# Atticuszz/GsplatLoc

Measured on AMD Instinct MI355X. Metric: Gaussians/s fwd+bwd @1M splats 1200x680, higher is better.
Workload: dtype f32

## Files before the change

### gsplatloc_amd/csrc/gsloc_common.h

```cpp
#pragma once
#include <hip/hip_runtime.h>
#include <stdint.h>

#include "../../include/gsloc_hip.h"

#define GSL_WAVE 64
#define GSL_ALPHA_MAX 0.999f
#define GSL_ALPHA_MIN (1.0f / 255.0f)
#define GSL_T_STOP 1e-4f
#define GSL_LOG2E 1.4426950408889634f

#define GSL_CHECK_LAUNCH()                                   \
  do {                                                       \
    hipError_t e__ = hipGetLastError();                      \
    if (e__ != hipSuccess) return GSL_ERR_HIP;               \
  } while (0)

namespace gsl {

int zero_u32(void* p, size_t n_dwords, hipStream_t st);

struct M3 {
  float m[9];
  __device__ __forceinline__ float& operator()(int r, int c) { return m[r * 3 + c]; }
  __device__ __forceinline__ float operator()(int r, int c) const { return m[r * 3 + c]; }
};

__device__ __forceinline__ M3 mul(const M3& a, const M3& b) {
  M3 o;
#pragma unroll
  for (int i = 0; i < 3; ++i)
#pragma unroll
    for (int j = 0; j < 3; ++j)
      o(i, j) = a(i, 0) * b(0, j) + a(i, 1) * b(1, j) + a(i, 2) * b(2, j);
  return o;
}
__device__ __forceinline__ M3 mul_bt(const M3& a, const M3& b) {
  M3 o;
#pragma unroll
  for (int i = 0; i < 3; ++i)
#pragma unroll
    for (int j = 0; j < 3; ++j)
      o(i, j) = a(i, 0) * b(j, 0) + a(i, 1) * b(j, 1) + a(i, 2) * b(j, 2);
  return o;
}
__device__ __forceinline__ M3 mul_at(const M3& a, const M3& b) {
  M3 o;
#pragma unroll
  for (int i = 0; i < 3; ++i)
#pragma unroll
    for (int j = 0; j < 3; ++j)
      o(i, j) = a(0, i) * b(0, j) + a(1, i) * b(1, j) + a(2, i) * b(2, j);
  return o;
}

__device__ __forceinline__ M3 quat_to_rotmat(float w, float x, float y, float z) {
  float inv = rsqrtf(w * w + x * x + y * y + z * z);
  w *= inv; x *= inv; y *= inv; z *= inv;
  M3 R;
  R(0, 0) = 1.f - 2.f * (y * y + z * z); R(0, 1) = 2.f * (x * y - w * z); R(0, 2) = 2.f * (x * z + w * y);
  R(1, 0) = 2.f * (x * y + w * z); R(1, 1) = 1.f - 2.f * (x * x + z * z); R(1, 2) = 2.f * (y * z - w * x);
  R(2, 0) = 2.f * (x * z - w * y); R(2, 1) = 2.f * (y * z + w * x); R(2, 2) = 1.f - 2.f * (x * x + y * y);
  return R;
}

__device__ __forceinline__ M3 quat_scale_to_covar(const float q[4], const float s[3]) {
  M3 R = quat_to_rotmat(q[0], q[1], q[2], q[3]);
  M3 M;
#pragma unroll
  for (int i = 0; i < 3; ++i)
#pragma unroll
    for (int j = 0; j < 3; ++j) M(i, j) = R(i, j) * s[j];
  return mul_bt(M, M);
}

struct Cam {
  M3 R;
  float t[3];
  float fx, fy, cx, cy;
};

__device__ __forceinline__ Cam load_cam(const float* __restrict__ V, const float* __restrict__ K) {
  Cam c;
#pragma unroll
  for (int i = 0; i < 3; ++i) {
#pragma unroll
    for (int j = 0; j < 3; ++j) c.R(i, j) = V[i * 4 + j];
    c.t[i] = V[i * 4 + 3];
  }
  c.fx = K[0]; c.fy = K[4]; c.cx = K[2]; c.cy = K[5];
  return c;
}

#define GSL_Q(arr, g) (arr)[(g)]
#ifndef GSL_NG
#define GSL_NG 4
#endif
#define GSL_HIT_SHIFT (32 - GSL_NG)
#define GSL_HIT_INDEX_MASK ((1u << GSL_HIT_SHIFT) - 1u)
#define GSL_CLAMP_DEPTH_WINDOW(nearp, farp)            \
  do {                                                 \
    if (!((nearp) >= 1.17549435e-38f)) (nearp) = 1.17549435e-38f; \
    if (!((farp) <= 3.40282347e+38f)) (farp) = 3.40282347e+38f;   \
  } while (0)
#define GSL_MAX_GAUSSIANS (1 << 26)
#ifndef GSL_XCD_SPANS
#define GSL_XCD_SPANS 0
#endif
__device__ __forceinline__ int xcd_span_item(int b, int n) {
#if GSL_XCD_SPANS
  const int x = b & 7, k = b >> 3, q = n >> 3, r = n & 7;
  return x * q + min(x, r) + k;
#else
  (void)n;
  return b;
#endif
}
#define GSL_TILE_OF_BLOCK() gsl::xcd_span_item((int)blockIdx.x, (int)gridDim.x)

__device__ __forceinline__ unsigned pack2h(float a, float b) {
  _Float16 ha = (_Float16)a, hb = (_Float16)b;
  return (unsigned)__builtin_bit_cast(unsigned short, ha) | ((unsigned)__builtin_bit_cast(unsigned short, hb) << 16);
}
__device__ __forceinline__ float h_lo(unsigned u) { return (float)__builtin_bit_cast(_Float16, (unsigned short)(u & 0xFFFFu)); }
__device__ __forceinline__ float h_hi(unsigned u) { return (float)__builtin_bit_cast(_Float16, (unsigned short)(u >> 16)); }

__device__ __forceinline__ void store_half_record(uint4* __restrict__ Qh, size_t i, float4 q0, float4 q1, float4 q2) {
  float rc = (q1.w > 0.f && q1.w < 6.0e4f) ? q1.w * 1.002f + 0.01f : q1.w;
  Qh[2 * i] = make_uint4(__float_as_uint(q0.x), __float_as_uint(q0.y), pack2h(q1.x, q1.y), pack2h(q1.z, rc));
  Qh[2 * i + 1] = make_uint4(pack2h(0.f, q0.w), pack2h(q2.x, q2.y), pack2h(q2.z, 0.f), __float_as_uint(q0.z));
}

__device__ __forceinline__ void load_record(const float4* __restrict__ Q0, const float4* __restrict__ Q1,
                                            const float4* __restrict__ Q2, const uint4* __restrict__ Qh, int g,
                                            bool want_rgb, float4& r0, float4& r1, float4& r2) {
  if (Qh) {
    uint4 lo = Qh[2 * (size_t)g], hi = Qh[2 * (size_t)g + 1];
    r0 = make_float4(__uint_as_float(lo.x), __uint_as_float(lo.y), __uint_as_float(hi.w), h_hi(hi.x));
    r1 = make_float4(h_lo(lo.z), h_hi(lo.z), h_lo(lo.w), h_hi(lo.w));
    r2 = make_float4(h_lo(hi.y), h_hi(hi.y), h_lo(hi.z), 0.f);
  } else {
    r0 = GSL_Q(Q0, g);
    r1 = GSL_Q(Q1, g);
    if (want_rgb) r2 = GSL_Q(Q2, g);
  }
}

__device__ __forceinline__ int32_t list_id(const int32_t* __restrict__ storage_of, uint64_t key) {
  uint32_t g = (uint32_t)key;
  return storage_of ? storage_of[g] : (int32_t)g;
}

template <int CTRL, int ROW_MASK = 0xF>
__device__ __forceinline__ float dpp_get(float v) {
  return __builtin_bit_cast(
      float, __builtin_amdgcn_update_dpp(0, __builtin_bit_cast(int, v), CTRL, ROW_MASK, 0xF, true));
}

__device__ __forceinline__ float wave_sum(float v) {
  v += dpp_get<0xB1>(v);
  v += dpp_get<0x4E>(v);
  v += dpp_get<0x141>(v);
  v += dpp_get<0x140>(v);
  v += dpp_get<0x142, 0xA>(v);
  v += dpp_get<0x143, 0xC>(v);
  return __builtin_bit_cast(float, __builtin_amdgcn_readlane(__builtin_bit_cast(int, v), 63));
}

__device__ __forceinline__ void cam_inverse(const Cam& cam, M3& Ri, float cp[3]) {
  const M3& R = cam.R;
  float c00 = R(1, 1) * R(2, 2) - R(1, 2) * R(2, 1);
  float c01 = R(1, 2) * R(2, 0) - R(1, 0) * R(2, 2);
  float c02 = R(1, 0) * R(2, 1) - R(1, 1) * R(2, 0);
  float det = R(0, 0) * c00 + R(0, 1) * c01 + R(0, 2) * c02;
  float id = 1.f / det;
  Ri(0, 0) = c00 * id; Ri(1, 0) = c01 * id; Ri(2, 0) = c02 * id;
  Ri(0, 1) = (R(0, 2) * R(2, 1) - R(0, 1) * R(2, 2)) * id;
  Ri(1, 1) = (R(0, 0) * R(2, 2) - R(0, 2) * R(2, 0)) * id;
  Ri(2, 1) = (R(0, 1) * R(2, 0) - R(0, 0) * R(2, 1)) * id;
  Ri(0, 2) = (R(0, 1) * R(1, 2) - R(0, 2) * R(1, 1)) * id;
  Ri(1, 2) = (R(0, 2) * R(1, 0) - R(0, 0) * R(1, 2)) * id;
  Ri(2, 2) = (R(0, 0) * R(1, 1) - R(0, 1) * R(1, 0)) * id;
#pragma unroll
  for (int k = 0; k < 3; ++k) cp[k] = -(Ri(k, 0) * cam.t[0] + Ri(k, 1) * cam.t[1] + Ri(k, 2) * cam.t[2]);
}

__device__ __forceinline__ float viewmat_from_totals(const float* tot, const float* __restrict__ V,
                                                     const float* __restrict__ Kmat) {
  float v = 0.f;
  if (threadIdx.x < 16) {
    int r = threadIdx.x >> 2, c = threadIdx.x & 3;
    if (r < 3) {
      Cam cam = load_cam(V, Kmat);
      M3 Ri;
      float cp[3];
      cam_inverse(cam, Ri, cp);
      float w = Ri(0, r) * tot[12] + Ri(1, r) * tot[13] + Ri(2, r) * tot[14];
      if (c < 3) v = tot[r * 3 + c] - w * cp[c];
      else v = tot[9 + r] - w;
    }
  }
  return v;
}

__device__ __forceinline__ float reduce_viewmat_rows(const float* __restrict__ partials, int nb,
                                                     const float* __restrict__ V, const float* __restrict__ Kmat,
                                                     float (*red)[15], float* tot) {
  int q = threadIdx.x & 3;
  const float4* rows = reinterpret_cast<const float4*>(partials) + q;
  float4 a0 = make_float4(0.f, 0.f, 0.f, 0.f), a1 = a0, a2 = a0, a3 = a0;
  int b = threadIdx.x >> 2;
  for (; b + 192 < nb; b += 256) {
    float4 x0 = rows[(size_t)b * 4], x1 = rows[(size_t)(b + 64) * 4], x2 = rows[(size_t)(b + 128) * 4],
           x3 = rows[(size_t)(b + 192) * 4];
    a0.x += x0.x; a0.y += x0.y; a0.z += x0.z; a0.w += x0.w;
    a1.x += x1.x; a1.y += x1.y; a1.z += x1.z; a1.w += x1.w;
    a2.x += x2.x; a2.y += x2.y; a2.z += x2.z; a2.w += x2.w;
    a3.x += x3.x; a3.y += x3.y; a3.z += x3.z; a3.w += x3.w;
  }
  for (; b < nb; b += 64) {
    float4 x0 = rows[(size_t)b * 4];
    a0.x += x0.x; a0.y += x0.y; a0.z += x0.z; a0.w += x0.w;
  }
  float v4[4] = {(a0.x + a1.x) + (a2.x + a3.x), (a0.y + a1.y) + (a2.y + a3.y), (a0.z + a1.z) + (a2.z + a3.z),
                 (a0.w + a1.w) + (a2.w + a3.w)};
  int lane = threadIdx.x & 63, wv = threadIdx.x >> 6;
#pragma unroll
  for (int c = 0; c < 4; ++c) {
    float x = v4[c];
#pragma unroll
    for (int o = 4; o < 64; o <<= 1) x += __shfl_xor(x, o, 64);
    if (lane < 4 && 4 * q + c < 15) red[wv][4 * q + c] = x;
  }
  __syncthreads();
  if (threadIdx.x < 15) tot[threadIdx.x] = red[0][threadIdx.x] + red[1][threadIdx.x] + red[2][threadIdx.x] + red[3][threadIdx.x];
  __syncthreads();
  return viewmat_from_totals(tot, V, Kmat);
}

__device__ __forceinline__ float reduce_viewmat_rows_wide(const float* __restrict__ partials, int nb,
                                                          const float* __restrict__ V, const float* __restrict__ Kmat,
                                                          float (*red)[15], float* tot) {
  int q = threadIdx.x & 3;
  const float4* rows = reinterpret_cast<const float4*>(partials) + q;
  float4 a0 = make_float4(0.f, 0.f, 0.f, 0.f), a1 = a0, a2 = a0, a3 = a0;
  int b = threadIdx.x >> 2;
  for (; b + 768 < nb; b += 1024) {
    float4 x0 = rows[(size_t)b * 4], x1 = rows[(size_t)(b + 256) * 4], x2 = rows[(size_t)(b + 512) * 4],
           x3 = rows[(size_t)(b + 768) * 4];
    a0.x += x0.x; a0.y += x0.y; a0.z += x0.z; a0.w += x0.w;
    a1.x += x1.x; a1.y += x1.y; a1.z += x1.z; a1.w += x1.w;
    a2.x += x2.x; a2.y += x2.y; a2.z += x2.z; a2.w += x2.w;
    a3.x += x3.x; a3.y += x3.y; a3.z += x3.z; a3.w += x3.w;
  }
  for (; b < nb; b += 256) {
    float4 x0 = rows[(size_t)b * 4];
    a0.x += x0.x; a0.y += x0.y; a0.z += x0.z; a0.w += x0.w;
  }
  float v4[4] = {(a0.x + a1.x) + (a2.x + a3.x), (a0.y + a1.y) + (a2.y + a3.y), (a0.z + a1.z) + (a2.z + a3.z),
                 (a0.w + a1.w) + (a2.w + a3.w)};
  int lane = threadIdx.x & 63, wv = threadIdx.x >> 6;
#pragma unroll
  for (int c = 0; c < 4; ++c) {
    float x = v4[c];
#pragma unroll
    for (int o = 4; o < 64; o <<= 1) x += __shfl_xor(x, o, 64);
    if (lane < 4 && 4 * q + c < 15) red[wv][4 * q + c] = x;
  }
  __syncthreads();
  if (threadIdx.x < 15) {
    float s = 0.f;
// ... 210 lines not shown
```

### gsplatloc_amd/csrc/raster_g16.hip

```cpp
#include <stdlib.h>
#include <string.h>

#include "gsloc_common.h"

namespace gsl {

__device__ __forceinline__ float g16_sel(unsigned long long m, float t, float f) {
  float r;
  asm("v_cndmask_b32_e64 %0, %1, %2, %3" : "=v"(r) : "v"(f), "v"(t), "s"(m));
  return r;
}

#define G16_M_LO8 0x00FF00FF00FF00FFull
#define G16_M_B2 0x0F0F0F0F0F0F0F0Full
#define G16_M_B1 0x3333333333333333ull
#define G16_M_B0 0x5555555555555555ull

constexpr int G16_NG = GSL_NG;
constexpr int G16_GL = 64 / G16_NG;
static_assert(G16_NG == 4 || G16_NG == 8, "pixel groups are DPP rows or half rows");

__device__ __forceinline__ float row_scatter8(const float (&v)[8]) {
  float n0, n1, n2, n3, m0, m1;
  asm volatile(
// ... 151 lines not shown
  const int pos_end = __builtin_amdgcn_readfirstlane(qhits ? 0 : (int)rs);
  while (pos > pos_end) {
    int staged = 0;
    int cnt[NG];
#pragma unroll
    for (int g = 0; g < NG; ++g) cnt[g] = 0;
    __syncthreads();
    while (pos > pos_end && staged <= GSL_QB - 64) {
      long long idx = (long long)(pos - 1 - lane);
      bool in = idx >= (long long)pos_end;
      unsigned nib = 0;
      int gid = 0;
      float4 r0 = make_float4(0.f, 0.f, 0.f, 0.f), r1 = r0, r2 = r0;
      if (in) {
        if (qhits) {
          unsigned e = qhits[idx];
          nib = e >> GSL_HIT_SHIFT;
          idx = (long long)(e & GSL_HIT_INDEX_MASK);
          gid = flatten_ids[idx];
          load_record(Q0, Q1, Q2, Qh, gid, RGB && CG == D, r0, r1, r2);
        } else {
          gid = flatten_ids[idx];
          load_record(Q0, Q1, Q2, Qh, gid, RGB && CG == D, r0, r1, r2);
          if (r1.w >= 0.f) {
            float rr = r1.w * r1.w;
#pragma unroll
            for (int g = 0; g < NG; ++g) {
              const int b = (NG == 8) ? (g >> 1) : g;
              const float cy = (NG == 8) ? 2.f * (float)(g & 1) + 1.f : 2.f, hy = (NG == 8) ? 0.5f : 1.5f;
              float ex = fmaxf(fabsf(r0.x - (qx0 + 4.f * (float)(b & 1) + 2.f)) - 1.5f, 0.f);
              float ey = fmaxf(fabsf(r0.y - (qy0 + 4.f * (float)(b >> 1) + cy)) - hy, 0.f);
              bool h = (ex * ex + ey * ey <= rr) && ((int)idx <= grp_final[g]);
              nib |= (h ? 1u : 0u) << g;
            }
          }
        }
      }
      unsigned long long R = __ballot(nib != 0);
      int slot = staged + __popcll(R & lt);
      unsigned pack[NG / 4];
#pragma unroll
      for (int w = 0; w < NG / 4; ++w) pack[w] = 0x0FFFFFFFu;
#pragma unroll
      for (int g = 0; g < NG; ++g) {
        unsigned long long Bg = __ballot(nib & (1u << g));
        if (__builtin_amdgcn_inverse_ballot_w64(Bg)) {
          int q = cnt[g] + __popcll(Bg & lt);
          sb.rlist[g][q] = (uint8_t)slot;
          pack[g >> 2] ^= (127u ^ (unsigned)q) << (7 * (g & 3));
        }
        cnt[g] += __popcll(Bg);
      }
      if (__builtin_amdgcn_inverse_ballot_w64(R)) {
        sb.id[slot] = gid;
        sb.s0[slot] = r0;
        sb.s1[slot] = make_float4(r1.x * (0.5f * GSL_LOG2E), r1.y * GSL_LOG2E, r1.z * (0.5f * GSL_LOG2E),
                                  __int_as_float((int)idx));
        if (RGB && CG == D) sb.s2[slot] = r2;
#pragma unroll
        for (int w = 0; w < NG / 4; ++w) sb.posn[w][slot] = pack[w];
      }
      staged += __popcll(R);
      pos -= 64;
    }
    if (staged == 0) continue;
    int kmax = 0, cnt_tot = 0, cnt_my = 0;
#pragma unroll
    for (int g = 0; g < NG; ++g) {
      kmax = max(kmax, cnt[g]);
      cnt_tot += cnt[g];
      cnt_my = (grp == g) ? cnt[g] : cnt_my;
    }
    G16_STAT(6, kmax);
    G16_STAT(7, cnt_tot);
    (void)cnt_tot;
    for (int k = cnt_my + p; k < kmax + 3; k += GL) mylist[k] = (uint8_t)GSL_QB;
    __syncthreads();
    constexpr int NU = (GSL_QB + 63) / 64;
    float mo[NU][NV];
#pragma unroll
    for (int u = 0; u < NU; ++u)
#pragma unroll
      for (int q = 0; q < NV; ++q) mo[u][q] = 0.f;
    auto trip = [&](int t, const float4& c0, const float4& c1, float4& r, float4& r2) {
      float dx = c0.x - px, dy = c0.y - py;
      float sigma = fmaf(c1.y * dx, dy, fmaf(c1.x * dx, dx, c1.z * dy * dy));
      float vis = __builtin_amdgcn_exp2f(-sigma);
      float opv = c0.w * vis;
      float alpha = fminf(GSL_ALPHA_MAX, opv);
      unsigned long long validm = __ballot(__float_as_int(c1.w) <= bin_final) & __ballot(sigma >= 0.f) &
                                  __ballot(alpha >= GSL_ALPHA_MIN);
      G16_STAT(0, 1);
      r = make_float4(0.f, 0.f, 0.f, 0.f);
      r2 = r;
      if (validm) {
        G16_STAT(1, 1);
#ifdef GSL_G16_STATS
        {
          int groups_hit = 0;
          for (int g = 0; g < NG; ++g) groups_hit += ((validm >> (GL * g)) & ((1ull << GL) - 1ull)) != 0;
          G16_STAT(3, groups_hit);
        }
#endif
        G16_STAT(5, __popcll(validm));
        unsigned long long capm = __ballot(opv <= GSL_ALPHA_MAX);
        float am = g16_sel(validm, alpha, 0.f);
        float ra = __builtin_amdgcn_rcpf(1.f - am);
        T *= ra;
        float fac = am * T;
        float cdot;
        if (CG == D) {
          cdot = 0.f;
          if (RGB) {
            float4 q2 = sb.s2[t];
            cdot = q2.x * vc[0] + q2.y * vc[1] + q2.z * vc[2];
          }
          if (DEPTH) cdot += c0.z * vc[D - 1];
        } else {
          cdot = c0.z * vc[D - 1];
        }
        float v_alpha = T * cdot - ra * Bp;
        Bp += fac * cdot;
        float w = g16_sel(validm & capm, vis, 0.f) * v_alpha;
        float val[NS];
        val[0] = w; val[1] = w * lx; val[2] = w * ly; val[3] = w * lxx; val[4] = w * lxy; val[5] = w * lyy;
        if (CG == D) {
#pragma unroll
          for (int ch = 0; ch < D; ++ch) val[6 + ch] = fac * vc[ch];
        } else {
          val[6] = fac * vc[D - 1];
        }
#pragma unroll
        for (int q = NV; q < NS; ++q) val[q] = 0.f;
        static_assert(NS != 8 || NV == 7, "the 8-value scatters treat value 7 as padding");
        if (NG == 8) {
          if (NS == 8) r = half_scatter8(reinterpret_cast<const float(&)[8]>(val));
          else half_scatter16(reinterpret_cast<const float(&)[16]>(val), r, r2);
        } else {
          if (NS == 8) r.x = row_scatter8(reinterpret_cast<const float(&)[8]>(val));
          else r.x = row_scatter16(reinterpret_cast<const float(&)[16]>(val));
        }
      }
    };
    auto put = [&](float* dst, const float4& r, const float4& r2) {
      if (NG == 8) {
        *reinterpret_cast<float4*>(dst) = r;
        if (NS == 16) *reinterpret_cast<float4*>(dst + 4) = r2;
      } else {
        *dst = r.x;
      }
    };
    for (int k0 = 0; k0 < kmax; k0 += LCAP) {
      const int k1 = min(k0 + LCAP, kmax);
      int t0 = mylist[k0], t1 = mylist[k0 + 1];
      float4 qa0 = sb.s0[t0], qa1 = sb.s1[t0];
      float4 ra = make_float4(0.f, 0.f, 0.f, 0.f), ra2 = ra, rb = ra, rb2 = ra;
      float* dst = mypair;
      for (int k = k0; k < k1; k += 2) {
        if (k > k0 && writer) put(dst - NS, rb, rb2);
        const int t2 = mylist[k + 2];
        const float4 qb0 = sb.s0[t1], qb1 = sb.s1[t1];
        trip(t0, qa0, qa1, ra, ra2);
        if (writer) put(dst, ra, ra2);
        const int t3 = mylist[k + 3];
        qa0 = sb.s0[t2];
        qa1 = sb.s1[t2];
        trip(t1, qb0, qb1, rb, rb2);
        t0 = t2;
        t1 = t3;
        dst += 2 * NS;
      }
      if (writer) put(dst - NS, rb, rb2);
      __syncthreads();
#pragma unroll
      for (int u = 0; u < NU; ++u) {
        int slot = lane + 64 * u;
        if (slot < staged) {
#pragma unroll
          for (int w = 0; w < NG / 4; ++w) {
            unsigned pk = sb.posn[w][slot];
#pragma unroll
            for (int g4 = 0; g4 < 4; ++g4) {
              const int g = 4 * w + g4;
              const unsigned q = ((pk >> (7 * g4)) & 127u) - (unsigned)k0;
              if (q < (unsigned)LCAP) {
                const float4* src = reinterpret_cast<const float4*>(&sb.pair[(g * LCAP + q) * NS]);
                float4 a = src[0], c = src[1];
                mo[u][0] += a.x; mo[u][1] += a.y; mo[u][2] += a.z; mo[u][3] += a.w;
                mo[u][4] += c.x; mo[u][5] += c.y; mo[u][6] += c.z;
                if (NV > 7) mo[u][7 < NV ? 7 : 0] += c.w;
                if (NS == 16) {
                  float4 e = src[2];
                  if (NV > 8) mo[u][8 < NV ? 8 : 0] += e.x;
                  if (NV > 9) mo[u][9 < NV ? 9 : 0] += e.y;
                }
              }
            }
          }
        }
      }
      __syncthreads();
    }
#pragma unroll
    for (int u = 0; u < NU; ++u) {
      int slot = lane + 64 * u;
      bool nz = false;
      float row[A];
#pragma unroll
      for (int k = 0; k < A; ++k) row[k] = 0.f;
      if (slot < staged) {
        {
          unsigned bits = 0u;
#pragma unroll
          for (int k = 0; k < NV; ++k) bits |= __float_as_uint(mo[u][k]);
          nz = (bits << 1) != 0u;
        }
        if (nz) {
          float4 r0 = sb.s0[slot], r1 = sb.s1[slot];
          float X = r0.x - tcx, Y = r0.y - tcy, S = mo[u][0];
          float Sx = X * S - mo[u][1], Sy = Y * S - mo[u][2];
          float Sxx = X * (X * S - 2.f * mo[u][1]) + mo[u][3];
          float Sxy = X * (Y * S - mo[u][2]) - Y * mo[u][1] + mo[u][4];
          float Syy = Y * (Y * S - 2.f * mo[u][2]) + mo[u][5];
          float no = -r0.w;
          r1.x *= 2.f / GSL_LOG2E; r1.y *= 1.f / GSL_LOG2E; r1.z *= 2.f / GSL_LOG2E;
          row[0] = no * (r1.x * Sx + r1.y * Sy);
          row[1] = no * (r1.y * Sx + r1.z * Sy);
          row[2] = 0.5f * no * Sxx;
          row[3] = no * Sxy;
          row[4] = 0.5f * no * Syy;
          row[5] = S;
          if (CG == D) {
#pragma unroll
            for (int ch = 0; ch < D; ++ch) row[6 + ch] = mo[u][6 + ch];
          } else {
            row[6 + D - 1] = mo[u][6];
          }
        }
      }
      float* packed = sb.pair;
      if (nz) {
#pragma unroll
        for (int k = 0; k < A; ++k) packed[lane * PP + k] = row[k];
      }
      unsigned long long mask = __ballot(nz);
      int cntz = __popcll(mask);
      if (nz) sb.nzlist[__popcll(mask & lt)] = (uint8_t)lane;
      __syncthreads();
      constexpr int RPI = 64 / A;
      const int arow = lane / A, f = lane - arow * A;
      for (int i0 = 0; i0 < cntz; i0 += RPI) {
        int gi = i0 + arow;
        if (gi < cntz && arow < RPI) {
          int sl = sb.nzlist[gi];
          const unsigned off = ((unsigned)sb.id[sl + 64 * u] << 6) | ((unsigned)f << 2);
          atomicAdd(reinterpret_cast<float*>(reinterpret_cast<char*>(vacc) + off), packed[sl * PP + f]);
        }
      }
      __syncthreads();
    }
  }
}

template <int D, bool ED, int CG, bool LONG>
__device__ __forceinline__ void qraster_bwd_item(
    QStage<D, CG>& sb, int b, int n_items, const float4* __restrict__ Q0, const float4* __restrict__ Q1,
    const float4* __restrict__ Q2, int W, int H, int tile_w, int ty0, const int32_t* __restrict__ tile_offsets,
    const int32_t* __restrict__ flatten_ids, long long capacity, const float* __restrict__ render,
    const float* __restrict__ alphas, const int32_t* __restrict__ last_ids, const float* __restrict__ v_render,
    const float* __restrict__ v_alphas, float* __restrict__ vacc, int row0, int row1, const uint4* __restrict__ Qh,
    const uint32_t* __restrict__ isect_hits, int32_t* __restrict__ isect_hit_counts, int long_min, LongWs lw,
    int32_t* __restrict__ rgb_flag, int32_t* __restrict__ clear_counts, int32_t* __restrict__ clear_state) {
  if (!LONG && (CG == 1 || D == 3) && clear_counts && (b & 3) == 0 && threadIdx.x == 0) {
    clear_counts[ty0 * tile_w + (b >> 2)] = 0;
    if (b == 0 && clear_state) *clear_state = 0;
  }
  const int wi = LONG ? b : xcd_span_item(b, n_items);
  const int quad = wi & 3, item = wi >> 2;
  int tile, sgm = 0, gseg = 0;
  if (LONG) {
    gseg = item;
    if (gseg >= lw.n_seg[0]) return;
    tile = lw.seg_tile[gseg];
    sgm = lw.seg_idx[gseg];
    if (tile < 0) return;
  } else {
    tile = ty0 * tile_w + item;
  }
  int tyi = tile / tile_w, txi = tile - tyi * tile_w;
  int lane = threadIdx.x, grp = lane >> 4, p = lane & 15;
  int j = txi * 16 + (quad & 1) * 8 + (grp & 1) * 4 + (p & 3);
  int i = tyi * 16 + (quad >> 1) * 8 + (grp >> 1) * 4 + (p >> 2);
  float px = (float)j + 0.5f, py = (float)i + 0.5f;
  bool inside = (i < H) && (j < W) && (i >= row0) && (i < row1);

  long long rs = tile_offsets[tile], re = tile_offsets[tile + 1];
  if (re > capacity) re = capacity;
  if (rs >= re) return;
  if (!LONG && long_min > 0 && re - rs > long_min) return;
  if (LONG) {
    rs += (long long)sgm * GSL_SEG;
    re = min(rs + (long long)GSL_SEG, re);
  }
  size_t pid = inside ? ((size_t)i * W + j) : 0;
  int bin_final = inside ? last_ids[pid] : -1;
  int quad_final = bin_final;
#pragma unroll
  for (int o = 32; o >= 1; o >>= 1) quad_final = max(quad_final, __shfl_xor(quad_final, o, 64));
  if ((long long)quad_final + 1 < re) re = (long long)quad_final + 1;
  if (rs >= re) return;
  float vc[D];
#pragma unroll
  for (int k = 0; k < D; ++k) vc[k] = inside ? v_render[pid * D + k] : 0.f;
  if (D == 4) {
    bool rgb_grad = (vc[0] != 0.f) || (vc[1] != 0.f) || (vc[2] != 0.f);
    bool any_rgb = __ballot(rgb_grad) != 0ull;
    if ((CG == 1) == any_rgb) {
      if (CG == 1 && rgb_flag && lane == 0) atomicOr(rgb_flag, 1);
      return;
    }
  }
  float Aimg = inside ? alphas[pid] : 0.f;
  float T_final = 1.f - Aimg;
  float va = inside ? v_alphas[pid] : 0.f;
  if (ED && inside) {
// ... 132 lines not shown
```

### gsplatloc_amd/csrc/raster_px.hip

```cpp
#include "gsloc_common.h"
#include "loss_dev.h"
#include "sort_dev.h"

namespace gsl {

template <int D>
struct PStage {
  float4 s0[256];
  float4 s1[256];
  float4 s2[(D >= 3) ? 256 : 1];
  uint16_t qlist[4][256];
  int qcnt[4][4];
};

template <int SHIFT = 0, typename Stage>
__device__ __forceinline__ int compact_quadrants(Stage& sb, int tid, bool valid_rec, float x, float y, float r,
                                                 float tile_x0, float tile_y0) {
  int lane = tid & 63, wv = tid >> 6;
  unsigned long long B[4];
#pragma unroll
  for (int q = 0; q < 4; ++q) {
    float cx = tile_x0 + 4.f + 8.f * (float)(q & 1), cy = tile_y0 + 4.f + 8.f * (float)(q >> 1);
    B[q] = __ballot(valid_rec) & __ballot(fabsf(x - cx) <= r + 3.5f) & __ballot(fabsf(y - cy) <= r + 3.5f);
  }
  if (lane < 4) {
    unsigned long long b = lane == 0 ? B[0] : (lane == 1 ? B[1] : (lane == 2 ? B[2] : B[3]));
    sb.qcnt[wv][lane] = __popcll(b);
  }
  __syncthreads();
  unsigned long long lt = (1ull << lane) - 1ull;
#pragma unroll
  for (int q = 0; q < 4; ++q) {
    if ((B[q] >> lane) & 1ull) {
      int base = 0;
      for (int w = 0; w < wv; ++w) base += sb.qcnt[w][q];
      sb.qlist[q][base + __popcll(B[q] & lt)] = (uint16_t)(tid << SHIFT);
    }
  }
  __syncthreads();
  return sb.qcnt[0][wv] + sb.qcnt[1][wv] + sb.qcnt[2][wv] + sb.qcnt[3][wv];
}

__device__ __forceinline__ void masked_mov2(unsigned& dlo, unsigned& dhi, unsigned long long value,
                                            unsigned long long lanes) {
  unsigned vlo = (unsigned)value, vhi = (unsigned)(value >> 32);
  unsigned long long saved;
  asm volatile("s_mov_b64 %2, exec\n\ts_and_b64 exec, %2, %5\n\tv_mov_b32 %0, %3\n\tv_mov_b32 %1, %4\n\ts_mov_b64 exec, %2"
               : "+v"(dlo), "+v"(dhi), "=&s"(saved)
               : "s"(vlo), "s"(vhi), "s"(lanes)
               : "scc");
}
template <bool BLOCKROWS = false>
__device__ __forceinline__ void pixel_masks(int lox, int hix, int loy, int hiy, int lane, unsigned& mlo, unsigned& mhi) {
  unsigned clo = 0, chi = 0, rlo = 0, rhi = 0;
  (void)lane;
#pragma unroll
  for (int v = 0; v < 8; ++v) {
    unsigned long long mc = __ballot(lox <= v) & __ballot(v <= hix);
    unsigned long long mr = __ballot(loy <= v) & __ballot(v <= hiy);
    if (BLOCKROWS) {
      masked_mov2(clo, chi, mc, (0x0000111100001111ull << (v & 3)) << (16 * (v >> 2)));
      masked_mov2(rlo, rhi, mr, (0x00000000000F000Full << (4 * (v & 3))) << (32 * (v >> 2)));
    } else {
      masked_mov2(clo, chi, mc, 0x0101010101010101ull << v);
      masked_mov2(rlo, rhi, mr, 0xFFull << (8 * v));
    }
  }
  mlo = clo & rlo;
  mhi = chi & rhi;
}

__device__ __forceinline__ unsigned group_or(unsigned v) {
  v |= (unsigned)__builtin_amdgcn_update_dpp(0, (int)v, 0xB1, 0xF, 0xF, true);
  v |= (unsigned)__builtin_amdgcn_update_dpp(0, (int)v, 0x4E, 0xF, 0xF, true);
  v |= (unsigned)__builtin_amdgcn_update_dpp(0, (int)v, 0x141, 0xF, 0xF, true);
#if GSL_NG == 4
  v |= (unsigned)__builtin_amdgcn_update_dpp(0, (int)v, 0x140, 0xF, 0xF, true);
#endif
  return v;
}

__device__ __forceinline__ unsigned sel_u32(unsigned long long m, unsigned t, unsigned f) {
  unsigned r;
  asm("v_cndmask_b32_e64 %0, %1, %2, %3" : "=v"(r) : "v"(f), "v"(t), "s"(m));
  return r;
}
__device__ __forceinline__ float sel_f32(unsigned long long m, float t, float f) {
  float r;
  asm("v_cndmask_b32_e64 %0, %1, %2, %3" : "=v"(r) : "v"(f), "v"(t), "s"(m));
  return r;
}

__device__ __forceinline__ int ffbl_raw(unsigned v) {
  int r;
  asm("v_ffbl_b32 %0, %1" : "=v"(r) : "v"(v));
  return r;
}

__device__ __forceinline__ float4 rec_at(const float4* arr, unsigned off) {
  return *reinterpret_cast<const float4*>(reinterpret_cast<const char*>(arr) + off);
}

__device__ __forceinline__ void box_range(float centre_rel, float r, int& lo, int& hi) {
  float l = ceilf(centre_rel - r), h = floorf(centre_rel + r);
  lo = (int)fmaxf(l, 0.f);
  hi = (int)fminf(h, 7.f);
}

template <int D, int MODE>
__device__ __forceinline__ void praster_walk(
    PStage<D>& sb, const float4* __restrict__ Q0, const float4* __restrict__ Q1, const float4* __restrict__ Q2,
    const uint4* __restrict__ Qh, const int32_t* __restrict__ flatten_ids, long long rs, long long re, int tid, float px,
    float py, int qx, int qy, int txi, int tyi, bool& done, float& T, float (&pix)[D], int& cur_idx,
    uint32_t* __restrict__ isect_hits, int& n_hits) {
  constexpr bool RGB = D >= 3;
  constexpr bool DEPTH = (D == 1) || (D == 4);
  const int lane = tid & 63, wv = tid >> 6;
  int nb = (int)((re - rs + 255) / 256);
  if (MODE == 1) isect_hits = nullptr;
  uint32_t* const qout = isect_hits ? isect_hits + 4 * rs + (long long)wv * (re - rs) : nullptr;
  n_hits = 0;
  unsigned long long DONE = __ballot(done);
  for (int b = 0; b < nb; ++b) {
    if (__syncthreads_and(DONE == ~0ull)) break;
    long long bstart = rs + (long long)b * 256;
    int bsize = (int)min((long long)256, re - bstart);
    float4 r0 = make_float4(0.f, 0.f, 0.f, 0.f), r1 = make_float4(0.f, 0.f, 0.f, -1.f);
    if (tid < bsize) {
      int g = flatten_ids[bstart + tid];
      float4 r2 = make_float4(0.f, 0.f, 0.f, 0.f);
      load_record(Q0, Q1, Q2, Qh, g, RGB && MODE == 0, r0, r1, r2);
      const float ca = r1.x * (0.5f * GSL_LOG2E), cb = r1.y * GSL_LOG2E, cc = r1.z * (0.5f * GSL_LOG2E);
      sb.s0[tid] = make_float4(r0.x, r0.y, ca, cb);
      if (RGB) {
        sb.s1[tid] = make_float4(cc, r0.w, r2.x, r2.y);
        sb.s2[tid] = make_float4(r2.z, r0.z, r1.w, 0.f);
      } else {
        sb.s1[tid] = make_float4(cc, r0.w, r0.z, r1.w);
      }
    } else {
      sb.s0[tid] = make_float4(0.f, 0.f, 0.f, 0.f);
      if (RGB) {
        sb.s1[tid] = make_float4(0.f, 0.f, 0.f, 0.f);
        sb.s2[tid] = make_float4(0.f, 0.f, -1.f, 0.f);
      } else {
        sb.s1[tid] = make_float4(0.f, 0.f, 0.f, -1.f);
      }
    }
    const int n = __builtin_amdgcn_readfirstlane(
        compact_quadrants<4>(sb, tid, tid < bsize, r0.x, r0.y, r1.w, (float)(txi * 16), (float)(tyi * 16)));
    for (int c = 0; c < n; c += 64) {
      if (DONE == ~0ull) break;
      int e = c + lane;
      int lox = 1, hix = 0, loy = 1, hiy = 0;
      if (e < n) {
        const unsigned off = sb.qlist[wv][e];
        float4 a0 = rec_at(sb.s0, off);
        float r = RGB ? rec_at(sb.s2, off).z : rec_at(sb.s1, off).w;
        box_range(a0.x - ((float)qx + 0.5f), r, lox, hix);
        box_range(a0.y - ((float)qy + 0.5f), r, loy, hiy);
      }
      unsigned mlo, mhi;
      pixel_masks<true>(lox, hix, loy, hiy, lane, mlo, mhi);
      mlo = sel_u32(DONE, 0u, mlo);
      mhi = sel_u32(DONE, 0u, mhi);
      unsigned cm[2] = {0u, 0u};
#pragma unroll
      for (int half = 0; half < 2; ++half) {
        unsigned m = half ? mhi : mlo;
        if (half) m = sel_u32(DONE, 0u, m);
        const uint16_t* const ql = &sb.qlist[wv][c + half * 32];
        unsigned long long ACT = __ballot(m != 0);
        if (ACT) do {
          const unsigned b0 = m & (0u - m);
          m ^= b0;
          const unsigned b1 = m & (0u - m);
          m ^= b1;
          const unsigned long long TWO = __ballot(b1 != 0u);
          const unsigned t0 = ql[ffbl_raw(b0)] & 0xFF0u;
          const unsigned t1 = ql[ffbl_raw(b1)] & 0xFF0u;
          float4 p0 = rec_at(sb.s0, t0), p1 = rec_at(sb.s1, t0);
          float4 u0 = rec_at(sb.s0, t1), u1 = rec_at(sb.s1, t1);
          float dx0 = p0.x - px, dy0 = p0.y - py, dx1 = u0.x - px, dy1 = u0.y - py;
          float sg0 = fmaf(p0.w * dx0, dy0, fmaf(p0.z * dx0, dx0, p1.x * dy0 * dy0));
          float sg1 = fmaf(u0.w * dx1, dy1, fmaf(u0.z * dx1, dx1, u1.x * dy1 * dy1));
          float al0 = fminf(GSL_ALPHA_MAX, p1.y * __builtin_amdgcn_exp2f(-sg0));
          float al1 = fminf(GSL_ALPHA_MAX, u1.y * __builtin_amdgcn_exp2f(-sg1));
          const unsigned long long OK0 = ACT & __ballot(sg0 >= 0.f) & __ballot(al0 >= GSL_ALPHA_MIN);
          const unsigned long long OK1 = TWO & __ballot(sg1 >= 0.f) & __ballot(al1 >= GSL_ALPHA_MIN);
          if (MODE == 1) {
            T *= 1.f - sel_f32(OK0, al0, 0.f);
            T *= 1.f - sel_f32(OK1, al1, 0.f);
            ACT = __ballot(m != 0);
            continue;
          }
          const unsigned long long S0R = __ballot(T * (1.f - al0) <= GSL_T_STOP);
          const unsigned long long STOP0 = OK0 & S0R, EFF0 = OK0 & ~S0R;
          const float a0 = sel_f32(EFF0, al0, 0.f);
          const float vis0 = a0 * T;
          const float T1 = T * (1.f - a0);
          const unsigned long long LIVE1 = OK1 & ~STOP0;
          const unsigned long long S1R = __ballot(T1 * (1.f - al1) <= GSL_T_STOP);
          const unsigned long long STOP1 = LIVE1 & S1R, EFF1 = LIVE1 & ~S1R;
          const float a1 = sel_f32(EFF1, al1, 0.f);
          const float vis1 = a1 * T1;
          T = T1 * (1.f - a1);
          if (RGB) {
            const float2 q20 = *reinterpret_cast<const float2*>(reinterpret_cast<const char*>(sb.s2) + t0);
            const float2 q21 = *reinterpret_cast<const float2*>(reinterpret_cast<const char*>(sb.s2) + t1);
            pix[0] += p1.z * vis0; pix[1] += p1.w * vis0; pix[2] += q20.x * vis0;
            if (DEPTH) pix[D - 1] += q20.y * vis0;
            pix[0] += u1.z * vis1; pix[1] += u1.w * vis1; pix[2] += q21.x * vis1;
            if (DEPTH) pix[D - 1] += q21.y * vis1;
          } else if (DEPTH) {
            pix[D - 1] += p1.z * vis0;
            pix[D - 1] += u1.z * vis1;
          }
          cm[half] |= sel_u32(EFF0, b0, 0u) | sel_u32(EFF1, b1, 0u);
          const unsigned long long STOPPED = STOP0 | STOP1;
          DONE |= STOPPED;
          m = sel_u32(STOPPED, 0u, m);
          ACT = __ballot(m != 0);
        } while (ACT);
      }
      {
        const bool any = (cm[0] | cm[1]) != 0u;
        const int pos = cm[1] ? 63 - __clz((int)cm[1]) : 31 - __clz((int)(cm[0] | 1u));
        const int tl = (sb.qlist[wv][c + pos] & 0xFF0u) >> 4;
        cur_idx = any ? (int)bstart + tl : cur_idx;
      }
      if (isect_hits) {
        unsigned rlo = group_or(cm[0]), rhi = group_or(cm[1]);
        unsigned nib = 0;
        unsigned long long Rm = 0ull;
#pragma unroll
        for (int g = 0; g < GSL_NG; ++g) {
          unsigned glo = (unsigned)__builtin_amdgcn_readlane((int)rlo, (64 / GSL_NG) * g);
          unsigned ghi = (unsigned)__builtin_amdgcn_readlane((int)rhi, (64 / GSL_NG) * g);
          unsigned long long gm = ((unsigned long long)ghi << 32) | glo;
          nib |= sel_u32(gm, 1u << g, 0u);
          Rm |= gm;
        }
        if (nib) qout[n_hits + __popcll(Rm & ((1ull << lane) - 1ull))] = (nib << GSL_HIT_SHIFT) | (unsigned)((int)bstart + (sb.qlist[wv][e] >> 4));
        n_hits += __popcll(Rm);
      }
    }
  }
  done = ((DONE >> lane) & 1ull) != 0ull;
}

struct TilePixel {
  int tyi, txi, qx, qy, i, j;
};
__device__ __forceinline__ TilePixel tile_pixel(int tile, int tile_w, int tid) {
  TilePixel t;
  int lane = tid & 63, wv = tid >> 6, grp = lane >> 4, pp = lane & 15;
  t.tyi = tile / tile_w;
  t.txi = tile - t.tyi * tile_w;
  t.qx = t.txi * 16 + (wv & 1) * 8;
  t.qy = t.tyi * 16 + (wv >> 1) * 8;
  t.j = t.qx + 4 * (grp & 1) + (pp & 3);
  t.i = t.qy + 4 * (grp >> 1) + (pp >> 2);
  return t;
}

struct FwdSort {
  uint64_t* bins;
  const int32_t* counts;
  int32_t* tile_offsets;
  int32_t* flatten_ids;
  int32_t* n_isects;
  int32_t* flags;
  int bin_cap;
  const int32_t* storage_of;
};
template <int SORT> struct FwdListPtr { typedef const int32_t* __restrict__ type; };
template <> struct FwdListPtr<2> { typedef const int32_t* type; };
template <> struct FwdListPtr<3> { typedef const int32_t* type; };

template <int D, bool ED, int SORT>
__global__ __launch_bounds__(256) __attribute__((amdgpu_waves_per_eu(SORT == 3 ? 4 : 6))) void k_praster_fwd(
    const float4* __restrict__ Q0, const float4* __restrict__ Q1, const float4* __restrict__ Q2, int W, int H,
    int tile_w, int ty0, typename FwdListPtr<SORT>::type tile_offsets, typename FwdListPtr<SORT>::type flatten_ids,
    long long capacity, float* __restrict__ render, float* __restrict__ alphas, int32_t* __restrict__ last_ids,
    int row0, int row1, const uint4* __restrict__ Qh, int32_t* __restrict__ clear_counts,
    int32_t* __restrict__ clear_state, uint32_t* __restrict__ isect_hits, int32_t* __restrict__ isect_hit_counts,
    int long_min, int n_tiles_total, FwdSort fs) {
  constexpr size_t SORT_BYTES = SORT ? (size_t)8 * 64 * (1 << SORT) * sizeof(uint64_t) : 0;
  constexpr size_t LDS_BYTES = sizeof(PStage<D>) > SORT_BYTES ? sizeof(PStage<D>) : SORT_BYTES;
  __shared__ __align__(16) unsigned char smem[LDS_BYTES];
  PStage<D>& sb = *reinterpret_cast<PStage<D>*>(smem);
  __shared__ int s_scan[5];
  int tile = ty0 * tile_w + GSL_TILE_OF_BLOCK();
  long long sorted_rs = 0, sorted_re = 0;
  if constexpr (SORT != 0) {
    const int tid = threadIdx.x, lane = tid & 63, wv = tid >> 6;
    int acc = prefix_count_share(fs.counts, tile, fs.bin_cap, tid);
#pragma unroll
    for (int o = 32; o >= 1; o >>= 1) acc += __shfl_xor(acc, o, 64);
    if (lane == 0) s_scan[wv] = acc;
    if (tid == 0) {
      int c_own = fs.counts[tile];
      s_scan[4] = min(c_own, fs.bin_cap);
      if (c_own > fs.bin_cap && fs.flags) { fs.flags[1] = 1; atomicMax(&fs.flags[2], c_own); }
    }
    __syncthreads();
    long long s0 = s_scan[0] + s_scan[1] + s_scan[2] + s_scan[3], e0 = s0 + s_scan[4];
    if (tid == 0) {
      fs.tile_offsets[tile] = (int32_t)s0;
      if (tile == n_tiles_total - 1) {
        fs.tile_offsets[tile + 1] = (int32_t)e0;
        if (fs.n_isects) fs.n_isects[0] = (int32_t)e0;
      }
    }
    if (e0 > capacity) e0 = capacity;
    int n = (int)max(e0 - s0, (long long)0);
    if (n > 256) {
      wg_sort_tile<SORT>(fs.bins + (size_t)tile * (size_t)fs.bin_cap, n, s0, tile, tid, reinterpret_cast<uint64_t*>(smem),
                         nullptr, fs.flatten_ids, nullptr, 0, fs.storage_of);
    } else if (n > 0 && wv == 0) {
      const uint64_t* src = fs.bins + (size_t)tile * (size_t)fs.bin_cap;
      uint64_t k[4];
#pragma unroll
      for (int r = 0; r < 4; ++r) k[r] = (lane * 4 + r < n) ? src[lane * 4 + r] : GSL_SORT_PAD;
      wave_sort_regs<2>(k, lane);
#pragma unroll
      for (int r = 0; r < 4; ++r)
        if (lane * 4 + r < n) fs.flatten_ids[s0 + lane * 4 + r] = list_id(fs.storage_of, k[r]);
    }
    __syncthreads();
    sorted_rs = s0;
    sorted_re = s0 + n;
  }
  if (clear_counts && threadIdx.x == 0) {
    clear_counts[tile] = 0;
    if (blockIdx.x == 0 && clear_state) *clear_state = 0;
  }
  if (isect_hit_counts && blockIdx.x == 0 && threadIdx.x == 0) isect_hit_counts[4 * n_tiles_total] = 0;
  int tid = threadIdx.x;
  TilePixel tp = tile_pixel(tile, tile_w, tid);
  int i = tp.i, j = tp.j;
  float px = (float)j + 0.5f, py = (float)i + 0.5f;
  bool inside = (i < H) && (j < W) && (i >= row0) && (i < row1);
  bool done = !inside;

  long long rs, re;
  if constexpr (SORT != 0) {
    rs = sorted_rs;
    re = sorted_re;
  } else {
    rs = tile_offsets[tile];
    re = tile_offsets[tile + 1];
    if (re > capacity) re = capacity;
    if (rs > re) rs = re;
    if (long_min > 0 && re - rs > long_min) return;
  }

  float T = 1.f;
  int cur_idx = 0;
  float pix[D];
#pragma unroll
  for (int k = 0; k < D; ++k) pix[k] = 0.f;
  int n_hits = 0;
  praster_walk<D, 0>(sb, Q0, Q1, Q2, Qh, flatten_ids, rs, re, tid, px, py, tp.qx, tp.qy, tp.txi, tp.tyi, done, T, pix,
                     cur_idx, isect_hits, n_hits);
  if (isect_hits && (tid & 63) == 0) isect_hit_counts[tile * 4 + (tid >> 6)] = n_hits;
  if (inside) {
    size_t pid = (size_t)i * W + j;
    float A = 1.f - T;
    alphas[pid] = A;
    if (ED) pix[D - 1] = pix[D - 1] / fmaxf(A, 1e-10f);
#pragma unroll
    for (int k = 0; k < D; ++k) render[pid * D + k] = pix[k];
    last_ids[pid] = cur_idx;
  }
}

template <int D, int PASS>
__global__ __launch_bounds__(256) void k_long_fwd(
    const float4* __restrict__ Q0, const float4* __restrict__ Q1, const float4* __restrict__ Q2, int W, int H,
    int tile_w, const int32_t* __restrict__ tile_offsets, const int32_t* __restrict__ flatten_ids, long long capacity,
    int row0, int row1, const uint4* __restrict__ Qh, uint32_t* __restrict__ isect_hits, LongWs w) {
  __shared__ PStage<D> sb;
  int g = blockIdx.x;
  if (g >= w.n_seg[0]) return;
  int tile = w.seg_tile[g], sgm = w.seg_idx[g];
  if (tile < 0) return;
  int tid = threadIdx.x;
  TilePixel tp = tile_pixel(tile, tile_w, tid);
  int i = tp.i, j = tp.j;
  float px = (float)j + 0.5f, py = (float)i + 0.5f;
  bool inside = (i < H) && (j < W) && (i >= row0) && (i < row1);
  long long rs = tile_offsets[tile], re = tile_offsets[tile + 1];
  if (re > capacity) re = capacity;
  long long ss = rs + (long long)sgm * GSL_SEG, se = min(ss + (long long)GSL_SEG, re);
  float pix[D];
#pragma unroll
  for (int k = 0; k < D; ++k) pix[k] = 0.f;
  size_t slot = (size_t)g * 256 + tid;
  if (PASS == 0) {
    float T = 1.f;
    int cur = 0;
    bool done = !inside;
    int nh = 0;
    praster_walk<D, 1>(sb, Q0, Q1, Q2, Qh, flatten_ids, ss, se, tid, px, py, tp.qx, tp.qy, tp.txi, tp.tyi, done, T, pix,
                       cur, nullptr, nh);
    w.P[slot] = T;
  } else {
    float T = 1.f;
    {
      const float* Pp = w.P + (size_t)(g - sgm) * 256 + tid;
      int s = 0;
      for (; s + 8 <= sgm; s += 8) {
        float v[8];
#pragma unroll
        for (int u = 0; u < 8; ++u) v[u] = Pp[(size_t)(s + u) * 256];
#pragma unroll
        for (int u = 0; u < 8; ++u) T *= v[u];
      }
      for (; s < sgm; ++s) T *= Pp[(size_t)s * 256];
    }
    bool dead = !inside || T <= GSL_T_STOP;
    bool done = dead;
    int cur = -1;
    int nh = 0;
    praster_walk<D, 0>(sb, Q0, Q1, Q2, Qh, flatten_ids, ss, se, tid, px, py, tp.qx, tp.qy, tp.txi, tp.tyi, done, T, pix,
                       cur, isect_hits, nh);
    if ((tid & 63) == 0) w.seg_qcnt[g * 4 + (tid >> 6)] = isect_hits ? nh : 0;
    w.Tend[slot] = dead ? 2.f : ((done && !dead) ? -T : T);
    w.last[slot] = cur;
#pragma unroll
    for (int k = 0; k < 4; ++k) w.C[slot * 4 + k] = (k < D) ? pix[k < D ? k : 0] : 0.f;
  }
}

template <int D, bool ED>
__global__ __launch_bounds__(1024) void k_long_combine(int W, int H, int tile_w, float* __restrict__ render,
                                                       float* __restrict__ alphas, int32_t* __restrict__ last_ids, int row0,
                                                       int row1, LongWs w) {
  __shared__ float4 s_pix[3][256];
  __shared__ float s_T[3][256];
  __shared__ int s_last[3][256];
  __shared__ int s_state[3][256];
  int g = blockIdx.x;
  if (g >= w.n_seg[0] || w.seg_idx[g] != 0) return;
  int tile = w.seg_tile[g], nseg = w.seg_cnt[g];
// ... 409 lines not shown
```

Measured before the change: 2.377 billion.

## Peel odd tail in raster loops and enable XCD-span tile mapping for forward

The forward pixel rasterizer's two-at-a-time gaussian loop is restructured so the pair loop runs only while both slots are valid, with a single-gaussian epilogue that avoids a wasted half-iteration. The g16 backward staging loop peels an odd leading element for non-RGB variants so the paired loop never processes a padded slot. The forward kernel also maps blocks to tiles in per-XCD contiguous spans by default, aiming for better L2 locality across chiplets. The extra branches add code size and register pressure, and the new tile mapping changes block scheduling order.

```diff
diff --git a/gsplatloc_amd/csrc/gsloc_common.h b/gsplatloc_amd/csrc/gsloc_common.h
--- a/gsplatloc_amd/csrc/gsloc_common.h
+++ b/gsplatloc_amd/csrc/gsloc_common.h
@@ -107,16 +107,20 @@
 #ifndef GSL_XCD_SPANS
 #define GSL_XCD_SPANS 0
 #endif
-__device__ __forceinline__ int xcd_span_item(int b, int n) {
-#if GSL_XCD_SPANS
-  const int x = b & 7, k = b >> 3, q = n >> 3, r = n & 7;
-  return x * q + min(x, r) + k;
-#else
-  (void)n;
+#ifndef GSL_XCD_SPANS_FWD
+#define GSL_XCD_SPANS_FWD 1
+#endif
+template <bool SPANS>
+__device__ __forceinline__ int xcd_item(int b, int n) {
+  if (SPANS) {
+    const int x = b & 7, k = b >> 3, q = n >> 3, r = n & 7;
+    return x * q + min(x, r) + k;
+  }
   return b;
-#endif
-}
+}
+__device__ __forceinline__ int xcd_span_item(int b, int n) { return xcd_item<GSL_XCD_SPANS != 0>(b, n); }
 #define GSL_TILE_OF_BLOCK() gsl::xcd_span_item((int)blockIdx.x, (int)gridDim.x)
+#define GSL_FWD_TILE_OF_BLOCK() gsl::xcd_item<GSL_XCD_SPANS_FWD != 0>((int)blockIdx.x, (int)gridDim.x)
 
 __device__ __forceinline__ unsigned pack2h(float a, float b) {
   _Float16 ha = (_Float16)a, hb = (_Float16)b;
diff --git a/gsplatloc_amd/csrc/raster_g16.hip b/gsplatloc_amd/csrc/raster_g16.hip
--- a/gsplatloc_amd/csrc/raster_g16.hip
+++ b/gsplatloc_amd/csrc/raster_g16.hip
@@ -327,25 +327,37 @@
     };
     for (int k0 = 0; k0 < kmax; k0 += LCAP) {
       const int k1 = min(k0 + LCAP, kmax);
-      int t0 = mylist[k0], t1 = mylist[k0 + 1];
-      float4 qa0 = sb.s0[t0], qa1 = sb.s1[t0];
       float4 ra = make_float4(0.f, 0.f, 0.f, 0.f), ra2 = ra, rb = ra, rb2 = ra;
       float* dst = mypair;
-      for (int k = k0; k < k1; k += 2) {
-        if (k > k0 && writer) put(dst - NS, rb, rb2);
-        const int t2 = mylist[k + 2];
-        const float4 qb0 = sb.s0[t1], qb1 = sb.s1[t1];
-        trip(t0, qa0, qa1, ra, ra2);
+      int ks = k0;
+      constexpr bool PEEL_ODD = (D != 3);
+      if (PEEL_ODD && ((k1 - k0) & 1)) {
+        const int t = mylist[k0];
+        const float4 q0 = sb.s0[t], q1 = sb.s1[t];
+        trip(t, q0, q1, ra, ra2);
         if (writer) put(dst, ra, ra2);
-        const int t3 = mylist[k + 3];
-        qa0 = sb.s0[t2];
-        qa1 = sb.s1[t2];
-        trip(t1, qb0, qb1, rb, rb2);
-        t0 = t2;
-        t1 = t3;
-        dst += 2 * NS;
-      }
-      if (writer) put(dst - NS, rb, rb2);
+        dst += NS;
+        ks = k0 + 1;
+      }
+      if (ks < k1) {
+        int t0 = mylist[ks], t1 = mylist[ks + 1];
+        float4 qa0 = sb.s0[t0], qa1 = sb.s1[t0];
+        for (int k = ks; k < k1; k += 2) {
+          if (k > ks && writer) put(dst - NS, rb, rb2);
+          const int t2 = mylist[k + 2];
+          const float4 qb0 = sb.s0[t1], qb1 = sb.s1[t1];
+          trip(t0, qa0, qa1, ra, ra2);
+          if (writer) put(dst, ra, ra2);
+          const int t3 = mylist[k + 3];
+          qa0 = sb.s0[t2];
+          qa1 = sb.s1[t2];
+          trip(t1, qb0, qb1, rb, rb2);
+          t0 = t2;
+          t1 = t3;
+          dst += 2 * NS;
+        }
+        if (writer) put(dst - NS, rb, rb2);
+      }
       __syncthreads();
 #pragma unroll
       for (int u = 0; u < NU; ++u) {
diff --git a/gsplatloc_amd/csrc/raster_px.hip b/gsplatloc_amd/csrc/raster_px.hip
--- a/gsplatloc_amd/csrc/raster_px.hip
+++ b/gsplatloc_amd/csrc/raster_px.hip
@@ -163,22 +163,23 @@
       unsigned mlo, mhi;
       pixel_masks<true>(lox, hix, loy, hiy, lane, mlo, mhi);
       mlo = sel_u32(DONE, 0u, mlo);
-      mhi = sel_u32(DONE, 0u, mhi);
       unsigned cm[2] = {0u, 0u};
 #pragma unroll
       for (int half = 0; half < 2; ++half) {
         unsigned m = half ? mhi : mlo;
         if (half) m = sel_u32(DONE, 0u, m);
         const uint16_t* const ql = &sb.qlist[wv][c + half * 32];
-        unsigned long long ACT = __ballot(m != 0);
-        if (ACT) do {
-          const unsigned b0 = m & (0u - m);
-          m ^= b0;
-          const unsigned b1 = m & (0u - m);
-          m ^= b1;
-          const unsigned long long TWO = __ballot(b1 != 0u);
-          const unsigned t0 = ql[ffbl_raw(b0)] & 0xFF0u;
-          const unsigned t1 = ql[ffbl_raw(b1)] & 0xFF0u;
+        unsigned b0 = m & (0u - m);
+        m ^= b0;
+        unsigned b1 = m & (0u - m);
+        m ^= b1;
+        unsigned long long ACT = __ballot(b0 != 0u);
+        unsigned long long TWO = __ballot(b1 != 0u);
+        while (TWO) {
+          unsigned q0 = ql[ffbl_raw(b0)], q1 = ql[ffbl_raw(b1)];
+          asm volatile("" : "+v"(q0), "+v"(q1));
+          const unsigned t0 = q0 & 0xFF0u;
+          const unsigned t1 = q1 & 0xFF0u;
           float4 p0 = rec_at(sb.s0, t0), p1 = rec_at(sb.s1, t0);
           float4 u0 = rec_at(sb.s0, t1), u1 = rec_at(sb.s1, t1);
           float dx0 = p0.x - px, dy0 = p0.y - py, dx1 = u0.x - px, dy1 = u0.y - py;
@@ -191,37 +192,67 @@
           if (MODE == 1) {
             T *= 1.f - sel_f32(OK0, al0, 0.f);
             T *= 1.f - sel_f32(OK1, al1, 0.f);
-            ACT = __ballot(m != 0);
-            continue;
+          } else {
+            const unsigned long long S0R = __ballot(T * (1.f - al0) <= GSL_T_STOP);
+            const unsigned long long STOP0 = OK0 & S0R, EFF0 = OK0 & ~S0R;
+            const float a0 = sel_f32(EFF0, al0, 0.f);
+            const float vis0 = a0 * T;
+            const float T1 = T * (1.f - a0);
+            const unsigned long long LIVE1 = OK1 & ~STOP0;
+            const unsigned long long S1R = __ballot(T1 * (1.f - al1) <= GSL_T_STOP);
+            const unsigned long long STOP1 = LIVE1 & S1R, EFF1 = LIVE1 & ~S1R;
+            const float a1 = sel_f32(EFF1, al1, 0.f);
+            const float vis1 = a1 * T1;
+            T = T1 * (1.f - a1);
+            if (RGB) {
+              const float2 q20 = *reinterpret_cast<const float2*>(reinterpret_cast<const char*>(sb.s2) + t0);
+              const float2 q21 = *reinterpret_cast<const float2*>(reinterpret_cast<const char*>(sb.s2) + t1);
+              pix[0] += p1.z * vis0; pix[1] += p1.w * vis0; pix[2] += q20.x * vis0;
+              if (DEPTH) pix[D - 1] += q20.y * vis0;
+              pix[0] += u1.z * vis1; pix[1] += u1.w * vis1; pix[2] += q21.x * vis1;
+              if (DEPTH) pix[D - 1] += q21.y * vis1;
+            } else if (DEPTH) {
+              pix[D - 1] += p1.z * vis0;
+              pix[D - 1] += u1.z * vis1;
+            }
+            cm[half] |= sel_u32(EFF0, b0, 0u) | sel_u32(EFF1, b1, 0u);
+            const unsigned long long STOPPED = STOP0 | STOP1;
+            DONE |= STOPPED;
+            m = sel_u32(STOPPED, 0u, m);
           }
-          const unsigned long long S0R = __ballot(T * (1.f - al0) <= GSL_T_STOP);
-          const unsigned long long STOP0 = OK0 & S0R, EFF0 = OK0 & ~S0R;
-          const float a0 = sel_f32(EFF0, al0, 0.f);
-          const float vis0 = a0 * T;
-          const float T1 = T * (1.f - a0);
-          const unsigned long long LIVE1 = OK1 & ~STOP0;
-          const unsigned long long S1R = __ballot(T1 * (1.f - al1) <= GSL_T_STOP);
-          const unsigned long long STOP1 = LIVE1 & S1R, EFF1 = LIVE1 & ~S1R;
-          const float a1 = sel_f32(EFF1, al1, 0.f);
-          const float vis1 = a1 * T1;
-          T = T1 * (1.f - a1);
-          if (RGB) {
-            const float2 q20 = *reinterpret_cast<const float2*>(reinterpret_cast<const char*>(sb.s2) + t0);
-            const float2 q21 = *reinterpret_cast<const float2*>(reinterpret_cast<const char*>(sb.s2) + t1);
-            pix[0] += p1.z * vis0; pix[1] += p1.w * vis0; pix[2] += q20.x * vis0;
-            if (DEPTH) pix[D - 1] += q20.y * vis0;
-            pix[0] += u1.z * vis1; pix[1] += u1.w * vis1; pix[2] += q21.x * vis1;
-            if (DEPTH) pix[D - 1] += q21.y * vis1;
-          } else if (DEPTH) {
-            pix[D - 1] += p1.z * vis0;
-            pix[D - 1] += u1.z * vis1;
+          b0 = m & (0u - m);
+          m ^= b0;
+          b1 = m & (0u - m);
+          m ^= b1;
+          ACT = __ballot(b0 != 0u);
+          TWO = __ballot(b1 != 0u);
+        }
+        if (ACT) {
+          const unsigned t0 = ql[ffbl_raw(b0)] & 0xFF0u;
+          float4 p0 = rec_at(sb.s0, t0), p1 = rec_at(sb.s1, t0);
+          float dx0 = p0.x - px, dy0 = p0.y - py;
+          float sg0 = fmaf(p0.w * dx0, dy0, fmaf(p0.z * dx0, dx0, p1.x * dy0 * dy0));
+          float al0 = fminf(GSL_ALPHA_MAX, p1.y * __builtin_amdgcn_exp2f(-sg0));
+          const unsigned long long OK0 = ACT & __ballot(sg0 >= 0.f) & __ballot(al0 >= GSL_ALPHA_MIN);
+          if (MODE == 1) {
+            T *= 1.f - sel_f32(OK0, al0, 0.f);
+          } else {
+            const unsigned long long S0R = __ballot(T * (1.f - al0) <= GSL_T_STOP);
+            const unsigned long long EFF0 = OK0 & ~S0R;
+            const float a0 = sel_f32(EFF0, al0, 0.f);
+            const float vis0 = a0 * T;
+            T = T * (1.f - a0);
+            if (RGB) {
+              const float2 q20 = *reinterpret_cast<const float2*>(reinterpret_cast<const char*>(sb.s2) + t0);
+              pix[0] += p1.z * vis0; pix[1] += p1.w * vis0; pix[2] += q20.x * vis0;
+              if (DEPTH) pix[D - 1] += q20.y * vis0;
+            } else if (DEPTH) {
+              pix[D - 1] += p1.z * vis0;
+            }
+            cm[half] |= sel_u32(EFF0, b0, 0u);
+            DONE |= OK0 & S0R;
           }
-          cm[half] |= sel_u32(EFF0, b0, 0u) | sel_u32(EFF1, b1, 0u);
-          const unsigned long long STOPPED = STOP0 | STOP1;
-          DONE |= STOPPED;
-          m = sel_u32(STOPPED, 0u, m);
-          ACT = __ballot(m != 0);
-        } while (ACT);
+        }
       }
       {
         const bool any = (cm[0] | cm[1]) != 0u;
@@ -291,7 +322,7 @@
   __shared__ __align__(16) unsigned char smem[LDS_BYTES];
   PStage<D>& sb = *reinterpret_cast<PStage<D>*>(smem);
   __shared__ int s_scan[5];
-  int tile = ty0 * tile_w + GSL_TILE_OF_BLOCK();
+  int tile = ty0 * tile_w + GSL_FWD_TILE_OF_BLOCK();
   long long sorted_rs = 0, sorted_re = 0;
   if constexpr (SORT != 0) {
     const int tid = threadIdx.x, lane = tid & 63, wv = tid >> 6;
```

New measurement: 2.394 billion (median of 6 runs). Within noise of the previous version (+0.7%).
